# voutcn/megahit

Hardware: NVIDIA H100
Metric: sorted (k+1)-mer edges/sec at k=27 on 150bp reads (higher is better)
Workload: dtype u32

## Files before the change

megahit_b200/csrc/mhb_count.cuh:

```cuda
#pragma once
#include <stdlib.h>
#include <string.h>

#include "mhb.h"
#include "mhb_kernels.cuh"

namespace mhb {

static constexpr int kReadsPerBatch = 64;
static constexpr int kStageWords = 4096;
static constexpr int kExtractThreads = 256;

struct ReadsView {
  const u32 *bin;
  u64 bin_words;
  u64 n_reads;
  u32 fixed_len;
  u32 fixed_stride;
  const u64 *rec_off;
  const u64 *edge_off;
  __device__ __forceinline__ u64 rec_start(u64 r) const { return fixed_len ? r * fixed_stride : rec_off[r]; }
};

template <class F>
__device__ __forceinline__ void for_each_read(const ReadsView &rv, F &&f) {
  __shared__ __align__(16) u32 s_stage[2][kStageWords];
  __shared__ __align__(8) u64 s_bar[2];
  const u32 tid = threadIdx.x, warp = tid >> 5;
  constexpr int NW = kExtractThreads / 32;
  const u64 n_batches = (rv.n_reads + kReadsPerBatch - 1) / kReadsPerBatch;
  if (tid == 0) {
    mbar_init(&s_bar[0], 1);
    mbar_init(&s_bar[1], 1);
    mbar_fence_init();
  }
  __syncthreads();

  auto geom = [&](u64 b, u64 &r0, u64 &r1, u64 &a0, u64 &a1) {
    r0 = b * kReadsPerBatch;
    r1 = r0 + kReadsPerBatch < rv.n_reads ? r0 + kReadsPerBatch : rv.n_reads;
    const u64 w0 = rv.rec_start(r0);
    const u64 w1 = r1 < rv.n_reads ? rv.rec_start(r1) : rv.bin_words;
    a0 = w0 & ~3ull;
    a1 = (w1 + 3) & ~3ull;
  };
  auto issue = [&](u64 b, int st) {
    u64 r0, r1, a0, a1;
    geom(b, r0, r1, a0, a1);
    if (a1 - a0 <= (u64)kStageWords && tid == 0) {
      const u32 bytes = (u32)(a1 - a0) * 4;
      mbar_expect_tx(&s_bar[st], bytes);
      bulk_g2s(&s_stage[st][0], rv.bin + a0, bytes, &s_bar[st]);
    }
  };

  u32 parity[2] = {0, 0};
  u64 b = blockIdx.x;
  int st = 0;
  if (b < n_batches) issue(b, 0);
  for (; b < n_batches; b += gridDim.x, st ^= 1) {
    const u64 nb = b + gridDim.x;
    if (nb < n_batches) issue(nb, st ^ 1);
    u64 r0, r1, a0, a1;
    geom(b, r0, r1, a0, a1);
    const bool staged = (a1 - a0) <= (u64)kStageWords;
    if (staged) {
      mbar_wait(&s_bar[st], parity[st]);
      parity[st] ^= 1;
    }
    for (u64 r = r0 + warp; r < r1; r += NW) {
      const u64 w = rv.rec_start(r);
      const u32 *rec = staged ? &s_stage[st][w - a0] : rv.bin + w;
      const u32 L = rec[0];
      f(r, rec + 1, div_ceil(L, 16), L);
    }
    __syncthreads();
  }
}

template <int W, int WR>
__global__ void __launch_bounds__(kExtractThreads)
    k_count_extract(ReadsView rv, u32 k, u32 *__restrict__ records, u64 *hist, int hist_byte) {
  __shared__ u32 s_hist[256];
  for (int i = threadIdx.x; i < 256; i += kExtractThreads) s_hist[i] = 0;
  const u32 lane = lane_id();
  const u32 K1 = k + 1;
  for_each_read(rv, [&](u64 r, const u32 *s, u32 nwords, u32 L) {
    if (L < K1) return;
    const u32 n_e = L - k;
    const u64 base = rv.fixed_len ? r * (u64)(rv.fixed_len - k) : rv.edge_off[r];
    for (u32 q0 = 0; q0 < n_e; q0 += 32) {
      const u32 q = q0 + lane;
      if (q < n_e) {
        u32 rec[WR], strand;
        make_count_record<W, WR>(s, nwords, L, k, q, rec, strand);
        st_rec<WR>(records, base + q, rec);
        if (hist) atomicAdd(&s_hist[rec_byte<WR>(rec, hist_byte)], 1u);
      }
    }
  });
  __syncthreads();
  if (hist)
    for (int i = threadIdx.x; i < 256; i += kExtractThreads)
      if (s_hist[i]) atomicAdd((unsigned long long *)&hist[i], (unsigned long long)s_hist[i]);
}

static __global__ void __launch_bounds__(kExtractThreads)
    k_count_extract_roll(ReadsView rv, u32 k, u32 *__restrict__ records, u64 *hist, int hist_byte) {
  __shared__ u32 s_hist[256];
  for (int i = threadIdx.x; i < 256; i += kExtractThreads) s_hist[i] = 0;
  const u32 lane = lane_id();
  const u32 K1 = k + 1;
  const u32 hshift = 8u * (u32)hist_byte;
  for_each_read(rv, [&](u64 r, const u32 *s, u32 nwords, u32 L) {
    if (L < K1) return;
    const u32 n_e = L - k;
    const u64 base = rv.fixed_len ? r * (u64)(rv.fixed_len - k) : rv.edge_off[r];
    for (u32 q0 = 0; q0 < n_e; q0 += 128) {
      const u32 q = q0 + 4 * lane;
      if (q < n_e) {
        u64 rec[4];
        u32 strand[4];
        make_count_records_roll<4>(s, nwords, L, k, q, rec, strand);
        const u32 cnt = n_e - q < 4u ? n_e - q : 4u;
#pragma unroll
        for (int j = 0; j < 4; ++j) {
          if ((u32)j < cnt) {
            reinterpret_cast<uint2 *>(records)[base + q + j] = make_uint2((u32)(rec[j] >> 32), (u32)rec[j]);
            if (hist) atomicAdd(&s_hist[(u32)(rec[j] >> hshift) & 255u], 1u);
          }
        }
      }
    }
  });
  __syncthreads();
  if (hist)
    for (int i = threadIdx.x; i < 256; i += kExtractThreads)
      if (s_hist[i]) atomicAdd((unsigned long long *)&hist[i], (unsigned long long)s_hist[i]);
}

template <int W, int WR, bool WRITE>
__global__ void __launch_bounds__(kExtractThreads)
    k_count_extract_range(ReadsView rv, u32 k, u32 lo, u32 hi, u64 *__restrict__ per_read, u32 *__restrict__ records,
                          u64 *hist, int hist_byte) {
  __shared__ u32 s_hist[256];
  for (int i = threadIdx.x; i < 256; i += kExtractThreads) s_hist[i] = 0;
  const u32 lane = lane_id();
  const u32 lt_mask = lanemask_lt();
  const u32 K1 = k + 1;
  for_each_read(rv, [&](u64 r, const u32 *s, u32 nwords, u32 L) {
    if (L < K1) {
      if (!WRITE && lane == 0) per_read[r] = 0;
      return;
    }
    const u32 n_e = L - k;
    u64 run = WRITE ? per_read[r] : 0ull;
    for (u32 q0 = 0; q0 < n_e; q0 += 32) {
      const u32 q = q0 + lane;
      u32 rec[WR], strand;
      bool in = false;
      if (q < n_e) {
        make_count_record<W, WR>(s, nwords, L, k, q, rec, strand);
        const u32 top = rec[0] >> 16;
        in = top >= lo && top <= hi;
      }
      const u32 mask = __ballot_sync(0xffffffffu, in);
      if (in) {
        if constexpr (WRITE) st_rec<WR>(records, run + __popc(mask & lt_mask), rec);
        if (hist) atomicAdd(&s_hist[rec_byte<WR>(rec, hist_byte)], 1u);
      }
      run += __popc(mask);
    }
    if (!WRITE && lane == 0) per_read[r] = run;
  });
  __syncthreads();
  if (hist)
    for (int i = threadIdx.x; i < 256; i += kExtractThreads)
      if (s_hist[i]) atomicAdd((unsigned long long *)&hist[i], (unsigned long long)s_hist[i]);
}

enum { kCountOwnHist = 0, kCountOwnWrite = 1 };
template <int W, int WR, int MODE>
__global__ void __launch_bounds__(kExtractThreads)
    k_count_extract_owners(ReadsView rv, u32 k, unsigned long long *__restrict__ hist16, OwnerSink sink,
                           const u32 *__restrict__ round_lo, const u32 *__restrict__ round_hi) {
  const u32 lane = lane_id(), lt = lanemask_lt();
  const u32 K1 = k + 1;
  for_each_read(rv, [&](u64, const u32 *s, u32 nwords, u32 L) {
    if (L < K1) return;
    const u32 n_e = L - k;
    for (u32 q0 = 0; q0 < n_e; q0 += 32) {
      const u32 q = q0 + lane;
      u32 rec[WR], strand;
      bool in = q < n_e;
      u32 b = 0xFFFFFFFFu;
      if (in) {
        make_count_record<W, WR>(s, nwords, L, k, q, rec, strand);
        b = rec[0] >> 16;
      }
      if constexpr (MODE == kCountOwnHist) {
        const u32 peers = __match_any_sync(0xffffffffu, b);
        if (in && lane == (u32)__ffs(peers) - 1) atomicAdd(hist16 + b, (unsigned long long)__popc(peers));
      } else {
        if (in) {
          const u32 o = __ldg(sink.owner + (b >> 8));
          in = b >= __ldg(round_lo + o) && b <= __ldg(round_hi + o);
        }
        const u32 mask = __ballot_sync(0xffffffffu, in);
        if (mask) sink.template put<WR>(in, rec, mask, lane, lt);
      }
    }
  });
}

template <int WR>
__device__ __forceinline__ bool same_edge(const u32 (&a)[WR], const u32 (&b)[WR]) {
  bool eq = true;
#pragma unroll
  for (int j = 0; j < WR; ++j) {
    const u32 m = (j == WR - 1) ? ~63u : ~0u;
    eq = eq && ((a[j] & m) == (b[j] & m));
  }
  return eq;
}

static constexpr int kMulHistSmem = 1024;

static __global__ void __launch_bounds__(1024) k_scan_u64(u64 *v, u64 nb, u64 *total_out) {
  __shared__ u64 s_w[33];
  __shared__ u64 s_carry;
  if (threadIdx.x == 0) s_carry = 0;
  __syncthreads();
  const u32 lane = lane_id(), warp = threadIdx.x >> 5;
  for (u64 base = 0; base < nb; base += 1024) {
    const u64 i = base + threadIdx.x;
    const u64 x = i < nb ? v[i] : 0;
    u64 inc = x;
#pragma unroll
    for (int d = 1; d < 32; d <<= 1) {
      u64 t = __shfl_up_sync(0xffffffffu, inc, d);
      if (lane >= (u32)d) inc += t;
    }
    if (lane == 31) s_w[warp] = inc;
    __syncthreads();
    if (warp == 0) {
      u64 w = s_w[lane], winc = w;
#pragma unroll
      for (int d = 1; d < 32; d <<= 1) {
        u64 t = __shfl_up_sync(0xffffffffu, winc, d);
        if (lane >= (u32)d) winc += t;
      }
      s_w[lane] = winc - w;
      if (lane == 31) s_w[32] = winc;
    }
    __syncthreads();
    if (i < nb) v[i] = s_carry + s_w[warp] + inc - x;
    __syncthreads();
    if (threadIdx.x == 0) s_carry += s_w[32];
    __syncthreads();
  }
  if (threadIdx.x == 0 && total_out) *total_out = s_carry;
}

struct TipsetHeader {
  u64 capacity;
  u64 filter_words;
  u32 fold;
  u32 filter_bits;
  u32 resident;
  u32 reserved;
};
static_assert(sizeof(TipsetHeader) == 32, "tip set header");
static constexpr u64 kTipFilterSmemWords = 224 * 1024 / 4;
static constexpr u64 kTipMul = 0x9E3779B97F4A7C15ull;

struct TipsetPlan {
  u64 capacity, filter_words;
  u32 fold, filter_bits, resident;
  __host__ __device__ u64 global_words() const { return fold * filter_words; }
  __host__ __device__ u64 folded_words() const { return fold > 1 ? filter_words : 0; }
};

inline TipsetPlan tipset_plan(u64 n_tip, const char *spec) {
  TipsetPlan p;
  p.capacity = 1024;
  while (p.capacity < 2 * n_tip) p.capacity <<= 1;
  char *end = nullptr;
  const unsigned long long forced = spec && *spec ? strtoull(spec, &end, 10) : 0ull;
  if (forced > 0 && end && *end == '\0') {
    p.filter_words = (forced + 3) & ~3ull;
// ... 688 lines not shown
```

megahit_b200/csrc/mhb_device.cu:

```cuda
#include <cuda_runtime.h>
#include <stdarg.h>
#include <stdio.h>
#include <stdlib.h>
#include <string.h>

#include "mhb.h"
#include "mhb_count.cuh"
#include "mhb_internal.h"
#include "mhb_mercy.cuh"
#include "mhb_s2s.cuh"
#include "mhb_common.cuh"

using namespace mhb;

static thread_local char g_err[1024] = "";
int mhb_set_error(int code, const char *fmt, ...) {
  va_list ap;
  va_start(ap, fmt);
  vsnprintf(g_err, sizeof(g_err), fmt, ap);
  va_end(ap);
  return code;
}
extern "C" const char *mhb_last_error(void) { return g_err; }
extern "C" const char *mhb_version(void) { return "megahit_b200 0.1 (sm_90a; formats of megahit v1.2.9)"; }
extern "C" int mhb_device_count(void) {
  int n = 0;
  if (cudaGetDeviceCount(&n) != cudaSuccess) {
    cudaGetLastError();
    return 0;
  }
  return n;
}
extern "C" void mhb_free(void *p) { free(p); }
unsigned long long g_mhb_launches = 0;
extern "C" uint64_t mhb_launch_count(void) { return g_mhb_launches; }


extern "C" uint32_t mhb_count_record_words(uint32_t k) { return count_record_words(k); }
extern "C" uint32_t mhb_words_per_edge(uint32_t k) { return words_per_edge(k); }
extern "C" uint32_t mhb_s2s_record_words(uint32_t k) { return s2s_record_words(k); }

extern "C" uint32_t mhb_count_sort_bytes(uint32_t k, uint8_t *bytes) {
  const u32 wr = count_record_words(k), total_bits = 32 * wr, key_bits = 2 * (k + 1);
  const u32 lo = (total_bits - key_bits) / 8;
  u32 n = 0;
  for (u32 b = lo; b < 4 * wr; ++b) bytes[n++] = (uint8_t)b;
  return n;
}
extern "C" uint32_t mhb_s2s_sort_bytes(uint32_t k, uint8_t *bytes) {
  const u32 w = s2s_record_words(k), total_bits = 32 * w, key_bits = 2 * k;
  const u32 lo = (total_bits - key_bits) / 8;
  u32 n = 0;
  for (u32 b = 2; b < 4 * w; ++b)
    if (b == 2 || b >= lo) bytes[n++] = (uint8_t)b;
  return n;
}


static int g_sm_count = 0;
static int g_bound_device = -1;
int mhb_sm_count() {
  if (!g_sm_count) {
    int dev = 0;
    cudaGetDevice(&dev);
    cudaDeviceGetAttribute(&g_sm_count, cudaDevAttrMultiProcessorCount, dev);
    if (g_sm_count <= 0) g_sm_count = 132;
    if (g_bound_device < 0) g_bound_device = dev;
  }
  return g_sm_count;
}

ReadsView make_reads_view(const mhb_dev_reads *r) {
  ReadsView v;
  v.bin = r->bin;
  v.bin_words = r->bin_words;
  v.n_reads = r->n_reads;
  v.fixed_len = r->fixed_len;
  v.fixed_stride = r->fixed_len ? 1 + div_ceil(r->fixed_len, 16) : 0;
  v.rec_off = r->rec_off;
  v.edge_off = r->edge_off;
  return v;
}

int check_reads(const mhb_dev_reads *r, uint32_t k) {
  if (!r || k < 1 || k > MHB_MAX_K) return mhb_set_error(MHB_ERR_ARG, "bad reads/k (k=%u)", k);
  if (r->n_reads && !r->bin) return mhb_set_error(MHB_ERR_ARG, "reads->bin is NULL");
  if (((uintptr_t)r->bin & 15) != 0) return mhb_set_error(MHB_ERR_ARG, "reads->bin must be 16-byte aligned");
  if (!r->fixed_len && r->n_reads && (!r->rec_off || !r->edge_off))
    return mhb_set_error(MHB_ERR_ARG, "variable-length reads need rec_off and edge_off");
  return MHB_OK;
}

static int grow_scratch(size_t bytes, void **out) {
  static void *buf[64] = {nullptr};
  static size_t cap[64] = {0};
  int dev = 0;
  CK(cudaGetDevice(&dev));
  if (dev < 0 || dev >= 64) return mhb_set_error(MHB_ERR_CUDA, "device index %d out of range", dev);
  if (cap[dev] < bytes) {
    CK(cudaDeviceSynchronize());
    if (buf[dev]) cudaFree(buf[dev]);
    buf[dev] = nullptr;
    cap[dev] = 0;
    const size_t want = (bytes + 4095) & ~(size_t)4095;
    CK(cudaMalloc(&buf[dev], want));
    cap[dev] = want;
  }
  *out = buf[dev];
  return MHB_OK;
}
static int scan64(cudaStream_t st, u64 *v, u64 n, u64 *total_dev, u64 *bsum);

static __global__ void k_check_fixed_len(const u32 *__restrict__ bin, u64 n_reads, u32 stride, u32 L, unsigned long long *flag) {
  bool bad = false;
  for (u64 r = (u64)blockIdx.x * blockDim.x + threadIdx.x; r < n_reads; r += (u64)gridDim.x * blockDim.x) bad |= bin[r * stride] != L;
  if (__any_sync(0xffffffffu, bad) && (threadIdx.x & 31) == 0) atomicOr(flag, 1ull);
}
extern "C" int mhb_check_fixed_len(void *stream, const uint32_t *bin_dev, uint64_t n_reads, uint32_t fixed_len, uint64_t *flag_dev) {
  if (n_reads == 0) return MHB_OK;
  if (!bin_dev || !flag_dev || !fixed_len) return mhb_set_error(MHB_ERR_ARG, "bad arguments");
  k_check_fixed_len<<<mhb_sm_count() * 8, 256, 0, (cudaStream_t)stream>>>(bin_dev, n_reads, 1 + div_ceil(fixed_len, 16), fixed_len,
                                                                     (unsigned long long *)flag_dev);
  CK_LAUNCH();
  return MHB_OK;
}

extern "C" int mhb_count_extract(void *stream, const mhb_dev_reads *reads, uint32_t k, uint32_t *records,
                                 uint64_t n_edges, uint64_t *hist256, int hist_byte) {
  if (int rc = check_reads(reads, k)) return rc;
  if (reads->n_reads == 0 || n_edges == 0) return MHB_OK;
  cudaStream_t st = (cudaStream_t)stream;
  const ReadsView rv = make_reads_view(reads);
  const u32 W = count_key_words(k), WR = count_record_words(k);
  const int grid = (int)grid_cap(rv.n_reads, kReadsPerBatch, 8);
  static const bool roll = getenv("MHB_EXTRACT_ROLL") && !strcmp(getenv("MHB_EXTRACT_ROLL"), "1");
  if (roll && W == 2 && WR == 2 && k + 1 >= 17) {
    k_count_extract_roll<<<grid, kExtractThreads, 0, st>>>(rv, k, records, hist256, hist_byte);
    CK_LAUNCH();
    return MHB_OK;
  }
#define M(WW)                                                                                              \
  if (W == WW && WR == WW)                                                                                 \
    k_count_extract<WW, WW><<<grid, kExtractThreads, 0, st>>>(rv, k, records, hist256, hist_byte);         \
  else if (W == WW && WR == WW + 1)                                                                        \
    k_count_extract<WW, WW + 1><<<grid, kExtractThreads, 0, st>>>(rv, k, records, hist256, hist_byte);     \
  else
  MHB_FOR_W(M) return mhb_set_error(MHB_ERR_ARG, "unsupported k=%u", k);
#undef M
  CK_LAUNCH();
  return MHB_OK;
}

extern "C" int mhb_count_extract_range(void *stream, const mhb_dev_reads *reads, uint32_t k, uint32_t lo, uint32_t hi,
                                       int write, uint64_t *per_read, uint32_t *records, uint64_t *hist256, int hist_byte,
                                       uint64_t *total_dev) {
  if (int rc = check_reads(reads, k)) return rc;
  if (lo > hi || hi > 65535) return mhb_set_error(MHB_ERR_ARG, "bad bucket range [%u, %u]", lo, hi);
  if (!per_read || (write && !records) || (!write && !total_dev)) return mhb_set_error(MHB_ERR_ARG, "null buffer");
  cudaStream_t st = (cudaStream_t)stream;
  if (reads->n_reads == 0) {
    if (!write) CK(cudaMemsetAsync(total_dev, 0, 8, st));
    return MHB_OK;
  }
  const ReadsView rv = make_reads_view(reads);
  const u32 W = count_key_words(k), WR = count_record_words(k);
  const int grid = (int)grid_cap(rv.n_reads, kReadsPerBatch, 8);
#define M2(WW, WRR)                                                                                                   \
  if (W == WW && WR == WRR) {                                                                                         \
    if (write)                                                                                                        \
      k_count_extract_range<WW, WRR, true><<<grid, kExtractThreads, 0, st>>>(rv, k, lo, hi, per_read, records, hist256, hist_byte); \
    else                                                                                                              \
      k_count_extract_range<WW, WRR, false><<<grid, kExtractThreads, 0, st>>>(rv, k, lo, hi, per_read, records, hist256, hist_byte); \
  } else
#define M(WW) M2(WW, WW) M2(WW, WW + 1)
  MHB_FOR_W(M) return mhb_set_error(MHB_ERR_ARG, "unsupported k=%u", k);
#undef M
#undef M2
  CK_LAUNCH();
  if (!write) {
    u64 *bsum = nullptr;
    if (int rc = grow_scratch(((rv.n_reads / kScanTile) + 2) * 8, (void **)&bsum)) return rc;
    if (int rc = scan64(st, per_read, rv.n_reads, total_dev, bsum)) return rc;
    CK(cudaMemcpyAsync(per_read + rv.n_reads, total_dev, 8, cudaMemcpyDeviceToDevice, st));
  }
  return MHB_OK;
}

extern "C" int mhb_count_extract_owners(void *stream, const mhb_dev_reads *reads, uint32_t k, uint64_t *hist16,
                                        const uint8_t *owner_of_byte, const uint64_t *owner_base, uint64_t *cursor_dev,
                                        const uint64_t *capacity_dev, const uint32_t *round_lo, const uint32_t *round_hi) {
  if (int rc = check_reads(reads, k)) return rc;
  if (!hist16 && (!owner_of_byte || !owner_base || !cursor_dev || !capacity_dev || !round_lo || !round_hi))
    return mhb_set_error(MHB_ERR_ARG, "bad args");
  if (reads->n_reads == 0) return MHB_OK;
  cudaStream_t st = (cudaStream_t)stream;
  const ReadsView rv = make_reads_view(reads);
  const u32 W = count_key_words(k), WR = count_record_words(k);
  const int grid = (int)grid_cap(rv.n_reads, kReadsPerBatch, 8);
  const OwnerSink sink{owner_of_byte, owner_base, (unsigned long long *)cursor_dev, capacity_dev};
  unsigned long long *h = (unsigned long long *)hist16;
#define M2(WW, WRR)                                                                                                         \
  if (W == WW && WR == WRR) {                                                                                               \
    if (hist16)                                                                                                             \
      k_count_extract_owners<WW, WRR, kCountOwnHist><<<grid, kExtractThreads, 0, st>>>(rv, k, h, sink, round_lo, round_hi);  \
    else                                                                                                                    \
      k_count_extract_owners<WW, WRR, kCountOwnWrite><<<grid, kExtractThreads, 0, st>>>(rv, k, h, sink, round_lo, round_hi); \
  } else
#define M(WW) M2(WW, WW) M2(WW, WW + 1)
  MHB_FOR_W(M) return mhb_set_error(MHB_ERR_ARG, "unsupported k=%u", k);
#undef M
#undef M2
  CK_LAUNCH();
  return MHB_OK;
}

extern "C" int mhb_count_solid(void *stream, const uint32_t *sorted_records, uint64_t n, uint32_t k, int32_t m,
                               uint32_t *edges_out, uint8_t *aux_out, uint64_t capacity_edges, uint64_t *mul_hist,
                               uint64_t *n_solid_out, void *scratch, size_t scratch_bytes) {
  if (k < 1 || k > MHB_MAX_K || !mul_hist || !n_solid_out) return mhb_set_error(MHB_ERR_ARG, "bad args");
  if (n == 0) return MHB_OK;
  const size_t need = mhb_count_solid_scratch_bytes(n);
  if (scratch_bytes < need) return mhb_set_error(MHB_ERR_ARG, "count scratch too small (%zu < %zu)", scratch_bytes, need);
  cudaStream_t st = (cudaStream_t)stream;
  const u32 WR = count_record_words(k);
  {
#define M(WW)                                                                                                          \
  if (WR == WW) {                                                                                                      \
    constexpr int CH = 32 * count3_ipl(WW);                                                                            \
    const u64 n_chunks = (n + CH - 1) / CH;                                                                            \
    if (n_chunks >= (1ull << 32)) return mhb_set_error(MHB_ERR_ARG, "too many records for one count launch");          \
    const u64 n_sblk = (n_chunks + kScanTile - 1) / kScanTile;                                                         \
    char *p = (char *)scratch;                                                                                         \
    u32 *ticket = (u32 *)p;                                                                                            \
    p += 256;                                                                                                          \
    uint2 *solid_list = (uint2 *)p;                                                                                    \
    p += pad256((size_t)n_chunks * CH * 8);                                                                            \
    u32 *chunk_count = (u32 *)p;                                                                                       \
    p += pad256((size_t)n_chunks * 4);                                                                                 \
    u64 *chunk_off = (u64 *)p;                                                                                         \
    p += pad256((size_t)n_chunks * 8);                                                                                 \
    u64 *bsum = (u64 *)p;                                                                                              \
    CK(cudaMemsetAsync(ticket, 0, 256, st));                                                                           \
    const size_t smem = (size_t)kCount3Warps * count3_warp_words(WW) * 4;                                              \
    static int bps = 0;                                                                                                \
    if (!bps) {                                                                                                        \
      CK(cudaFuncSetAttribute(k_count_lanes<WW>, cudaFuncAttributeMaxDynamicSharedMemorySize, (int)smem));             \
      CK(cudaOccupancyMaxActiveBlocksPerMultiprocessor(&bps, k_count_lanes<WW>, kCount3Warps * 32, smem));             \
      if (bps < 1) bps = 1;                                                                                            \
    }                                                                                                                  \
    u64 grid = (u64)sm_count() * bps;                                                                                  \
    if (grid > (n_chunks + kCount3Warps - 1) / kCount3Warps) grid = (n_chunks + kCount3Warps - 1) / kCount3Warps;      \
    k_count_lanes<WW><<<(unsigned)grid, kCount3Warps * 32, smem, st>>>(sorted_records, n, k, m, (u32)n_chunks, ticket,  \
                                                                      solid_list, chunk_count, mul_hist);             \
    CK_LAUNCH();                                                                                                       \
    k_scan32_sums<<<(unsigned)n_sblk, kScanThreads, 0, st>>>(chunk_count, n_chunks, bsum);                             \
    CK_LAUNCH();                                                                                                       \
    k_scan_u64<<<1, 1024, 0, st>>>(bsum, n_sblk, n_solid_out);                                                         \
    CK_LAUNCH();                                                                                                       \
    k_scan32_apply<<<(unsigned)n_sblk, kScanThreads, 0, st>>>(chunk_count, n_chunks, bsum, chunk_off);                 \
    CK_LAUNCH();                                                                                                       \
    k_count_write<WW><<<grid_cap(n_chunks, 8, 16), 256, 0, st>>>(sorted_records, k, (u32)n_chunks, solid_list, chunk_count, \
                                                    chunk_off, edges_out, aux_out, capacity_edges);                   \
  }
    MHB_FOR_WR(M)
#undef M
    CK_LAUNCH();
    return MHB_OK;
  }
  return mhb_set_error(MHB_ERR_ARG, "unsupported k=%u", k);
}

extern "C" size_t mhb_count_solid_scratch_bytes(uint64_t n) {
  return (size_t)(n + 1024) * 8 + (size_t)(n / 128 + 2) * 12 + (size_t)(n / 128 / kScanTile + 2) * 8 + 4096;
}

static TipsetPlan tipset_plan_env(uint64_t n_tip) { return tipset_plan(n_tip, getenv("MHB_TIPSET_FILTER")); }

extern "C" size_t mhb_tipset_bytes(uint64_t n_tip_edges, uint32_t k) {
  const TipsetPlan p = tipset_plan_env(n_tip_edges);
  return sizeof(TipsetHeader) + (p.global_words() + p.folded_words()) * 4 +
         p.capacity * (size_t)tipset_slot_words(count_key_words(k)) * 4;
}

static int small_scratch(unsigned long long **out) {
  static unsigned long long *buf[64] = {nullptr};
  int dev = 0;
  CK(cudaGetDevice(&dev));
  if (dev < 0 || dev >= 64) return mhb_set_error(MHB_ERR_CUDA, "device index %d out of range", dev);
  if (!buf[dev]) CK(cudaMalloc((void **)&buf[dev], 256));
  *out = buf[dev];
  return MHB_OK;
}

extern "C" int mhb_count_tip_edges(void *stream, const uint8_t *aux, uint64_t n_solid, uint64_t *n_tip_host) {
  cudaStream_t st = (cudaStream_t)stream;
  unsigned long long *d = nullptr;
  *n_tip_host = 0;
  if (n_solid == 0) return MHB_OK;
  if (int rc = small_scratch(&d)) return rc;
  CK(cudaMemsetAsync(d, 0, 8, st));
  k_count_tips<<<sm_count() * 4, 256, 0, st>>>(aux, n_solid, d);
  CK_LAUNCH();
  CK(cudaMemcpyAsync(n_tip_host, d, 8, cudaMemcpyDeviceToHost, st));
// ... 475 lines not shown
```

megahit_b200/csrc/mhb_kernels.cuh:

```cuda
#pragma once
#include <cuda_runtime.h>
#include <stdint.h>

#include "mhb_bits.cuh"

namespace mhb {

static constexpr u32 kSentinel = 4;


template <int W, int WR>
MHB_HD void make_count_record(const u32 *s, u32 nwords, u32 L, u32 k, u32 q, u32 (&rec)[WR], u32 &strand) {
  const u32 K1 = k + 1;
  u32 prev_pkg, next_pkg;
  bool st;
  if constexpr (W == 2) {
    const u32 w0 = q >> 4, sh = (q & 15) * 2;
    const u32 x0 = s[w0];
    const u32 x1 = (w0 + 1 < nwords) ? s[w0 + 1] : 0u;
    const u32 x2 = (w0 + 2 < nwords) ? s[w0 + 2] : 0u;
    const u32 pi = q + K1;
    const u32 pw = ((pi >> 4) == w0 + 1) ? x1 : x2;
    prev_pkg = (pi < L) ? ((pw >> (30 - 2 * (pi & 15))) & 3u) : kSentinel;
    const u32 nwd = (q & 15) ? x0 : (q ? s[w0 - 1] : 0u);
// ... 67 lines not shown

template <int W>
MHB_HD void make_s2s_record(const u32 *s, u32 nwords, u32 L, u32 k, u32 strand, u32 offset, u32 mult,
                            u32 (&rec)[W]) {
  const u32 nc = k - ((offset + k > L) ? 1u : 0u);
  const u32 counting = (offset > 0 && offset + k <= L) ? mult : 0u;
  u32 prev;
  if (strand == 0) {
    prev = offset == 0 ? kSentinel : base_at(s, offset - 1);
    load_sub<W>(s, nwords, offset, nc, rec);
  } else {
    prev = offset == 0 ? kSentinel : 3u - base_at(s, L - offset);
    int off2 = (int)L - (int)k - (int)offset;
    if (off2 < 0) off2 = 0;
    u32 S[W], T[W];
    load_sub<W>(s, nwords, (u32)off2, nc, S);
    reverse_sub<W>(S, nc, T);
    complement_sub<W>(T, nc, rec);
  }
  rec[W - 1] |= ((nc == k) ? 1u : 0u) << 19;
  rec[W - 1] |= prev << 16;
  rec[W - 1] |= 65535u - counting;
}

template <int W>
MHB_HD u64 s2s_local_key(const u32 (&r)[W], u32 k) {
  u32 w2 = 0;
  if constexpr (W >= 3) w2 = r[2];
  const u64 top = ((u64)r[0] << 48) | ((u64)r[1] << 16) | (w2 >> 16);
  const u32 kb = 2 * k - 16;
  const u64 flags = (r[W - 1] >> 16) & 15u;
  return (top & ~(~0ull >> kb)) | (flags << (60 - kb));
}

#if defined(__CUDACC__)
template <int WR>
__device__ __forceinline__ void ld_rec(const u32 *base, u64 idx, u32 (&r)[WR]) {
  if constexpr (WR % 4 == 0) {
    const uint4 *p = reinterpret_cast<const uint4 *>(base + idx * WR);
#pragma unroll
    for (int j = 0; j < WR / 4; ++j) {
      const uint4 v = p[j];
      r[4 * j] = v.x;
      r[4 * j + 1] = v.y;
      r[4 * j + 2] = v.z;
      r[4 * j + 3] = v.w;
    }
  } else if constexpr (WR % 2 == 0) {
    const uint2 *p = reinterpret_cast<const uint2 *>(base + idx * WR);
#pragma unroll
    for (int j = 0; j < WR / 2; ++j) {
      const uint2 v = p[j];
      r[2 * j] = v.x;
      r[2 * j + 1] = v.y;
    }
  } else {
    const u32 *p = base + idx * WR;
#pragma unroll
    for (int j = 0; j < WR; ++j) r[j] = p[j];
  }
}
template <int WR>
__device__ __forceinline__ void st_rec(u32 *base, u64 idx, const u32 (&r)[WR]) {
  if constexpr (WR % 4 == 0) {
    uint4 *p = reinterpret_cast<uint4 *>(base + idx * WR);
#pragma unroll
    for (int j = 0; j < WR / 4; ++j) p[j] = make_uint4(r[4 * j], r[4 * j + 1], r[4 * j + 2], r[4 * j + 3]);
  } else if constexpr (WR % 2 == 0) {
    uint2 *p = reinterpret_cast<uint2 *>(base + idx * WR);
#pragma unroll
    for (int j = 0; j < WR / 2; ++j) p[j] = make_uint2(r[2 * j], r[2 * j + 1]);
  } else {
    u32 *p = base + idx * WR;
#pragma unroll
    for (int j = 0; j < WR; ++j) p[j] = r[j];
  }
}

template <int WR>
__device__ __forceinline__ u32 rec_byte(const u32 (&r)[WR], int b) {
  return (pick<WR>(r, (u32)(WR - 1 - (b >> 2))) >> (8 * (b & 3))) & 255u;
}

template <int W>
__global__ void k_bucket_bounds(const u32 *__restrict__ recs, u64 n, u64 *__restrict__ bounds) {
  const u32 b = blockIdx.x * blockDim.x + threadIdx.x;
  if (b > 65536u) return;
  u64 lo = 0, hi = n;
  while (lo < hi) {
    const u64 mid = (lo + hi) >> 1;
    if ((recs[mid * W] >> 16) < b) lo = mid + 1;
    else hi = mid;
  }
  bounds[b] = lo;
}

__device__ __forceinline__ u32 lane_id() { return threadIdx.x & 31; }
__device__ __forceinline__ u32 lanemask_lt() {
  u32 m;
  asm("mov.u32 %0, %%lanemask_lt;" : "=r"(m));
  return m;
}

struct OwnerSink {
  const uint8_t *owner;
  const u64 *base;
  unsigned long long *cursor;
  const u64 *capacity;
  template <int W>
  __device__ __forceinline__ void put(bool in, const u32 (&rec)[W], u32, u32 lane, u32 lt) const {
    const u32 o = in ? (u32)__ldg(owner + (rec[0] >> 24)) : 0xFFFFFFFFu;
    const u32 peers = __match_any_sync(0xffffffffu, o);
    if (!in) return;
    const u32 leader = (u32)__ffs(peers) - 1;
    unsigned long long at = 0;
    if (lane == leader) at = atomicAdd(cursor + o, (unsigned long long)__popc(peers));
    at = __shfl_sync(peers, at, leader);
    const u64 pos = at + __popc(peers & lt);
    if (pos < capacity[o]) st_rec<W>(reinterpret_cast<u32 *>(base[o]), pos, rec);
  }
};

__device__ __forceinline__ u32 smem_u32(const void *p) { return (u32)__cvta_generic_to_shared(p); }
__device__ __forceinline__ void mbar_init(u64 *bar, u32 count) {
  asm volatile("mbarrier.init.shared::cta.b64 [%0], %1;" ::"r"(smem_u32(bar)), "r"(count) : "memory");
}
__device__ __forceinline__ void mbar_fence_init() {
  asm volatile("fence.mbarrier_init.release.cluster;" ::: "memory");
  asm volatile("fence.proxy.async.shared::cta;" ::: "memory");
}
__device__ __forceinline__ void mbar_expect_tx(u64 *bar, u32 bytes) {
  asm volatile("mbarrier.arrive.expect_tx.shared::cta.b64 _, [%0], %1;" ::"r"(smem_u32(bar)), "r"(bytes)
               : "memory");
}
__device__ __forceinline__ void bulk_g2s(void *dst, const void *src, u32 bytes, u64 *bar) {
  asm volatile("cp.async.bulk.shared::cluster.global.mbarrier::complete_tx::bytes [%0], [%1], %2, [%3];" ::"r"(
                   smem_u32(dst)),
               "l"(src), "r"(bytes), "r"(smem_u32(bar))
               : "memory");
}
__device__ __forceinline__ bool mbar_try_wait(u64 *bar, u32 parity) {
  u32 ok;
  asm volatile(
      "{\n\t.reg .pred p;\n\tmbarrier.try_wait.parity.shared::cta.b64 p, [%1], %2;\n\tselp.u32 %0, 1, 0, p;\n\t}"
      : "=r"(ok)
      : "r"(smem_u32(bar)), "r"(parity)
      : "memory");
  return ok != 0;
}
__device__ __forceinline__ void mbar_wait(u64 *bar, u32 parity) {
  while (!mbar_try_wait(bar, parity)) {
  }
}

__device__ __forceinline__ u64 ld_relaxed(const u64 *p) {
  u64 v;
  asm volatile("ld.relaxed.gpu.global.u64 %0, [%1];" : "=l"(v) : "l"(p) : "memory");
  return v;
}
__device__ __forceinline__ void st_relaxed(u64 *p, u64 v) {
  asm volatile("st.relaxed.gpu.global.u64 [%0], %1;" ::"l"(p), "l"(v) : "memory");
}

static constexpr u64 kLbPartial = 1ull << 62, kLbInclusive = 2ull << 62, kLbStatusMask = 3ull << 62;
static constexpr u64 kLbValueMask = (1ull << 54) - 1;
__host__ __device__ inline u64 lb_epoch(u32 e) { return (u64)(e & 255u) << 54; }

template <int THREADS>
__device__ __forceinline__ u32 block_excl_scan(u32 v, u32 *s_warp , u32 &total) {
  const u32 lane = lane_id(), warp = threadIdx.x >> 5;
  u32 inc = v;
#pragma unroll
  for (int d = 1; d < 32; d <<= 1) {
    u32 t = __shfl_up_sync(0xffffffffu, inc, d);
    if (lane >= (u32)d) inc += t;
  }
  if (lane == 31) s_warp[warp] = inc;
  __syncthreads();
  if (warp == 0) {
    u32 w = lane < THREADS / 32 ? s_warp[lane] : 0u;
    u32 winc = w;
#pragma unroll
    for (int d = 1; d < 32; d <<= 1) {
      u32 t = __shfl_up_sync(0xffffffffu, winc, d);
      if (lane >= (u32)d) winc += t;
    }
    if (lane < THREADS / 32) s_warp[lane] = winc - w;
    if (lane == 31) s_warp[THREADS / 32] = winc;
  }
  __syncthreads();
  u32 res = s_warp[warp] + inc - v;
  total = s_warp[THREADS / 32];
  __syncthreads();
  return res;
}
#endif

}
```

Measured before the change: 18.75 billion.

## Rewrite count extraction with TMA staging, warp-private output buffers and bulk stores

Replaces the extract kernels with one kernel that keeps a 3-stage ring of input batches, loaded by cp.async.bulk with full/empty mbarriers. Each warp writes its records into a double-buffered shared-memory output area and flushes them to global memory with bulk shared-to-global copies, fixing up the unaligned head and tail. Each warp also takes a contiguous range of reads, and for k=27 the rolling path processes two reads per warp step, one per half-warp. The goal is to turn scattered 8-byte stores into large coalesced bulk writes, overlap input loads with compute, and improve lane utilisation on 150bp reads; the cost is much more shared memory, which can lower occupancy, and more complex synchronisation.

```diff
diff --git a/megahit_b200/csrc/mhb_count.cuh b/megahit_b200/csrc/mhb_count.cuh
--- a/megahit_b200/csrc/mhb_count.cuh
+++ b/megahit_b200/csrc/mhb_count.cuh
@@ -78,64 +78,211 @@
   }
 }
 
+static constexpr int kExtThreads = 256;
+static constexpr int kExtWarps = kExtThreads / 32;
+static constexpr int kExtInStages = 3;
+static constexpr int kExtInWords = 2048;
+static constexpr int kExtOutBytes = 3072;
+static constexpr int kExtOutStride = kExtOutBytes + 16;
+static constexpr int kExtHistBytes = 1024, kExtBarBytes = 64;
+static constexpr int kExtSmemBytes =
+    kExtHistBytes + kExtBarBytes + kExtInStages * kExtInWords * 4 + kExtWarps * 2 * kExtOutStride;
+static_assert(2 * kExtInStages * 8 <= kExtBarBytes && kExtOutStride % 16 == 0, "extract shared-memory layout");
+
+__host__ __device__ inline u32 extract_reads_per_batch(u64 n_reads, u64 bin_words, u32 fixed_stride) {
+  const u64 stride = fixed_stride ? fixed_stride : (n_reads ? (bin_words + n_reads - 1) / n_reads : 1);
+  const u64 room = fixed_stride ? (u64)kExtInWords - 6 : (u64)kExtInWords / 2;
+  const u64 r = stride ? room / stride : room;
+  return r < 1 ? 1u : (u32)r;
+}
+
 template <int W, int WR>
-__global__ void __launch_bounds__(kExtractThreads)
-    k_count_extract(ReadsView rv, u32 k, u32 *__restrict__ records, u64 *hist, int hist_byte) {
-  __shared__ u32 s_hist[256];
-  for (int i = threadIdx.x; i < 256; i += kExtractThreads) s_hist[i] = 0;
-  const u32 lane = lane_id();
+__global__ void __launch_bounds__(kExtThreads)
+    k_count_extract(ReadsView rv, u32 k, u32 rpb, u32 *__restrict__ records, u64 *hist, int hist_byte) {
+  extern __shared__ __align__(16) unsigned char ext_smem[];
+  constexpr bool kRoll = W == 2 && WR == 2;
+  constexpr u32 SR = kRoll ? 128 : 32;
+  constexpr u32 CAP = kExtOutBytes / (4 * WR);
+  constexpr u32 kPairEdges = 128;
+  static_assert(CAP >= SR && (!kRoll || CAP >= 2 * kPairEdges), "an output buffer holds a warp step");
+  u32 *s_hist = reinterpret_cast<u32 *>(ext_smem);
+  u64 *full = reinterpret_cast<u64 *>(ext_smem + kExtHistBytes);
+  u64 *empty = full + kExtInStages;
+  u32 *s_in = reinterpret_cast<u32 *>(ext_smem + kExtHistBytes + kExtBarBytes);
+  const u32 tid = threadIdx.x, lane = lane_id(), warp = tid >> 5;
+  unsigned char *s_out = ext_smem + kExtHistBytes + kExtBarBytes + kExtInStages * kExtInWords * 4 + warp * 2 * kExtOutStride;
+  for (int i = tid; i < 256; i += kExtThreads) s_hist[i] = 0;
+  if (tid == 0) {
+    for (int s = 0; s < kExtInStages; ++s) {
+      mbar_init(&full[s], 1);
+      mbar_init(&empty[s], kExtWarps);
+    }
+    mbar_fence_init();
+  }
+  __syncthreads();
+
   const u32 K1 = k + 1;
-  for_each_read(rv, [&](u64 r, const u32 *s, u32 nwords, u32 L) {
-    if (L < K1) return;
-    const u32 n_e = L - k;
-    const u64 base = rv.fixed_len ? r * (u64)(rv.fixed_len - k) : rv.edge_off[r];
-    for (u32 q0 = 0; q0 < n_e; q0 += 32) {
-      const u32 q = q0 + lane;
-      if (q < n_e) {
-        u32 rec[WR], strand;
-        make_count_record<W, WR>(s, nwords, L, k, q, rec, strand);
-        st_rec<WR>(records, base + q, rec);
-        if (hist) atomicAdd(&s_hist[rec_byte<WR>(rec, hist_byte)], 1u);
-      }
-    }
-  });
+  const u64 n_batches = (rv.n_reads + rpb - 1) / rpb;
+  auto geom = [&](u64 b, u64 &r0, u64 &r1, u64 &a0, u64 &a1) {
+    r0 = b * rpb;
+    r1 = r0 + rpb < rv.n_reads ? r0 + rpb : rv.n_reads;
+    const u64 w0 = rv.rec_start(r0);
+    const u64 w1 = r1 < rv.n_reads ? rv.rec_start(r1) : rv.bin_words;
+    a0 = w0 & ~3ull;
+    a1 = (w1 + 3) & ~3ull;
+  };
+  auto issue = [&](u64 i) {
+    const u64 b = blockIdx.x + i * gridDim.x;
+    if (b >= n_batches) return;
+    const u32 st = (u32)(i % kExtInStages);
+    if (i >= (u64)kExtInStages) mbar_wait(&empty[st], (u32)((i / kExtInStages - 1) & 1));
+    u64 r0, r1, a0, a1;
+    geom(b, r0, r1, a0, a1);
+    if (a1 - a0 <= (u64)kExtInWords) {
+      const u32 bytes = (u32)(a1 - a0) * 4;
+      mbar_expect_tx(&full[st], bytes);
+      bulk_g2s(s_in + st * kExtInWords, rv.bin + a0, bytes, &full[st]);
+    } else {
+      mbar_expect_tx(&full[st], 0);
+    }
+  };
+
+  u32 cur = 0, n = 0, o = 0;
+  u64 d0 = 0;
+  auto flush = [&]() {
+    const u32 *sw = reinterpret_cast<const u32 *>(s_out + cur * kExtOutStride + o);
+    u32 *g = records + d0 * WR;
+    const u32 nw = n * WR;
+    const u32 h = min(((16u - o) & 15u) >> 2, nw);
+    const u32 body = (nw - h) & ~3u;
+    const u32 tail = nw - h - body;
+    fence_proxy_async_smem();
+    __syncwarp();
+    if (lane == 0) {
+      if (body) {
+        bulk_s2g(g + h, sw + h, body * 4);
+        bulk_commit();
+        bulk_wait_read<1>();
+      } else {
+        bulk_wait_read<0>();
+      }
+    }
+    if (lane < h) g[lane] = sw[lane];
+    else if (lane >= 4 && lane - 4 < tail) g[h + body + lane - 4] = sw[h + body + lane - 4];
+    __syncwarp();
+    cur ^= 1;
+    n = 0;
+  };
+  auto reserve = [&](u64 dst, u32 cnt) -> u32 * {
+    if (n && (dst != d0 + n || n + cnt > CAP)) flush();
+    if (n == 0) {
+      d0 = dst;
+      o = (u32)(reinterpret_cast<uintptr_t>(records + dst * WR) & 15u);
+    }
+    return reinterpret_cast<u32 *>(s_out + cur * kExtOutStride + o);
+  };
+
+  if (tid == 0)
+    for (int i = 0; i < kExtInStages - 1; ++i) issue(i);
+  for (u64 i = 0;; ++i) {
+    const u64 b = blockIdx.x + i * gridDim.x;
+    if (b >= n_batches) break;
+    if (tid == 0) issue(i + kExtInStages - 1);
+    const u32 st = (u32)(i % kExtInStages);
+    mbar_wait(&full[st], (u32)((i / kExtInStages) & 1));
+    u64 r0, r1, a0, a1;
+    geom(b, r0, r1, a0, a1);
+    const bool staged = a1 - a0 <= (u64)kExtInWords;
+    const u64 nr = r1 - r0;
+    const u64 my0 = r0 + nr * warp / kExtWarps, my1 = r0 + nr * (warp + 1) / kExtWarps;
+    auto read_words = [&](u64 r) -> const u32 * {
+      const u64 w = rv.rec_start(r);
+      return staged ? s_in + st * kExtInWords + (w - a0) : rv.bin + w;
+    };
+    for (u64 r = my0; r < my1; ++r) {
+      const u32 *rec0 = read_words(r);
+      const u32 L = rec0[0];
+      if constexpr (kRoll) {
+        if (r + 1 < my1) {
+          const u32 *rec1 = read_words(r + 1);
+          const u32 L1 = rec1[0];
+          const u32 ne0 = L >= K1 ? L - k : 0u, ne1 = L1 >= K1 ? L1 - k : 0u;
+          if (ne0 <= kPairEdges && ne1 <= kPairEdges) {
+            const u32 cnt = ne0 + ne1;
+            if (cnt) {
+              const u64 dst = rv.fixed_len ? r * (u64)(rv.fixed_len - k) : rv.edge_off[r];
+              u32 *buf = reserve(dst, cnt);
+              const u32 half = lane >> 4;
+              const u32 Lh = half ? L1 : L, ne = half ? ne1 : ne0;
+              const u32 q = 8 * (lane & 15);
+              if (q < ne) {
+                u64 rec[8];
+                u32 strand[8];
+                make_count_records_roll<8>((half ? rec1 : rec0) + 1, div_ceil(Lh, 16), Lh, k, q, rec, strand);
+                const u32 c = ne - q < 8u ? ne - q : 8u;
+                const u32 at = (u32)(dst - d0) + (half ? ne0 : 0u) + q;
+                const u32 hshift = 8u * (u32)hist_byte;
+#pragma unroll
+                for (int j = 0; j < 8; ++j) {
+                  if ((u32)j < c) {
+                    reinterpret_cast<uint2 *>(buf)[at + j] = make_uint2((u32)(rec[j] >> 32), (u32)rec[j]);
+                    if (hist) red_shared_add(&s_hist[(u32)(rec[j] >> hshift) & 255u], 1u);
+                  }
+                }
+              }
+              n += cnt;
+            }
+            ++r;
+            continue;
+          }
+        }
+      }
+      if (L < K1) continue;
+      const u32 *s = rec0 + 1;
+      const u32 nwords = div_ceil(L, 16);
+      const u32 n_e = L - k;
+      const u64 base = rv.fixed_len ? r * (u64)(rv.fixed_len - k) : rv.edge_off[r];
+      for (u32 q0 = 0; q0 < n_e; q0 += SR) {
+        const u32 cnt = n_e - q0 < SR ? n_e - q0 : SR;
+        const u64 dst = base + q0;
+        u32 *buf = reserve(dst, cnt);
+        const u32 at = (u32)(dst - d0);
+        if constexpr (kRoll) {
+          const u32 q = q0 + 4 * lane;
+          if (q < n_e) {
+            u64 rec[4];
+            u32 strand[4];
+            make_count_records_roll<4>(s, nwords, L, k, q, rec, strand);
+            const u32 c = n_e - q < 4u ? n_e - q : 4u;
+            const u32 hshift = 8u * (u32)hist_byte;
+#pragma unroll
+            for (int j = 0; j < 4; ++j) {
+              if ((u32)j < c) {
+                reinterpret_cast<uint2 *>(buf)[at + 4 * lane + j] = make_uint2((u32)(rec[j] >> 32), (u32)rec[j]);
+                if (hist) red_shared_add(&s_hist[(u32)(rec[j] >> hshift) & 255u], 1u);
+              }
+            }
+          }
+        } else {
+          const u32 q = q0 + lane;
+          if (q < n_e) {
+            u32 rec[WR], strand;
+            make_count_record<W, WR>(s, nwords, L, k, q, rec, strand);
+            st_rec<WR>(buf, at + lane, rec);
+            if (hist) red_shared_add(&s_hist[rec_byte<WR>(rec, hist_byte)], 1u);
+          }
+        }
+        n += cnt;
+      }
+    }
+    __syncwarp();
+    if (lane == 0) mbar_arrive(&empty[st]);
+  }
+  if (n) flush();
+  if (lane == 0) bulk_wait_all();
   __syncthreads();
   if (hist)
-    for (int i = threadIdx.x; i < 256; i += kExtractThreads)
-      if (s_hist[i]) atomicAdd((unsigned long long *)&hist[i], (unsigned long long)s_hist[i]);
-}
-
-static __global__ void __launch_bounds__(kExtractThreads)
-    k_count_extract_roll(ReadsView rv, u32 k, u32 *__restrict__ records, u64 *hist, int hist_byte) {
-  __shared__ u32 s_hist[256];
-  for (int i = threadIdx.x; i < 256; i += kExtractThreads) s_hist[i] = 0;
-  const u32 lane = lane_id();
-  const u32 K1 = k + 1;
-  const u32 hshift = 8u * (u32)hist_byte;
-  for_each_read(rv, [&](u64 r, const u32 *s, u32 nwords, u32 L) {
-    if (L < K1) return;
-    const u32 n_e = L - k;
-    const u64 base = rv.fixed_len ? r * (u64)(rv.fixed_len - k) : rv.edge_off[r];
-    for (u32 q0 = 0; q0 < n_e; q0 += 128) {
-      const u32 q = q0 + 4 * lane;
-      if (q < n_e) {
-        u64 rec[4];
-        u32 strand[4];
-        make_count_records_roll<4>(s, nwords, L, k, q, rec, strand);
-        const u32 cnt = n_e - q < 4u ? n_e - q : 4u;
-#pragma unroll
-        for (int j = 0; j < 4; ++j) {
-          if ((u32)j < cnt) {
-            reinterpret_cast<uint2 *>(records)[base + q + j] = make_uint2((u32)(rec[j] >> 32), (u32)rec[j]);
-            if (hist) atomicAdd(&s_hist[(u32)(rec[j] >> hshift) & 255u], 1u);
-          }
-        }
-      }
-    }
-  });
-  __syncthreads();
-  if (hist)
-    for (int i = threadIdx.x; i < 256; i += kExtractThreads)
+    for (int i = tid; i < 256; i += kExtThreads)
       if (s_hist[i]) atomicAdd((unsigned long long *)&hist[i], (unsigned long long)s_hist[i]);
 }
 
diff --git a/megahit_b200/csrc/mhb_device.cu b/megahit_b200/csrc/mhb_device.cu
--- a/megahit_b200/csrc/mhb_device.cu
+++ b/megahit_b200/csrc/mhb_device.cu
@@ -125,6 +125,20 @@
   return MHB_OK;
 }
 
+template <int W, int WR>
+static int launch_extract(cudaStream_t st, const ReadsView &rv, u32 k, u32 *records, u64 *hist256, int hist_byte) {
+  CK(cudaFuncSetAttribute(k_count_extract<W, WR>, cudaFuncAttributeMaxDynamicSharedMemorySize, kExtSmemBytes));
+  int per_sm = 0;
+  CK(cudaOccupancyMaxActiveBlocksPerMultiprocessor(&per_sm, k_count_extract<W, WR>, kExtThreads, kExtSmemBytes));
+  const u32 rpb = extract_reads_per_batch(rv.n_reads, rv.bin_words, rv.fixed_stride);
+  const u64 n_batches = (rv.n_reads + rpb - 1) / rpb;
+  const u64 cap = (u64)mhb_sm_count() * (u64)(per_sm > 0 ? per_sm : 1);
+  const int grid = (int)(n_batches < cap ? n_batches : cap);
+  k_count_extract<W, WR><<<grid, kExtThreads, kExtSmemBytes, st>>>(rv, k, rpb, records, hist256, hist_byte);
+  CK_LAUNCH();
+  return MHB_OK;
+}
+
 extern "C" int mhb_count_extract(void *stream, const mhb_dev_reads *reads, uint32_t k, uint32_t *records,
                                  uint64_t n_edges, uint64_t *hist256, int hist_byte) {
   if (int rc = check_reads(reads, k)) return rc;
@@ -132,23 +146,14 @@
   cudaStream_t st = (cudaStream_t)stream;
   const ReadsView rv = make_reads_view(reads);
   const u32 W = count_key_words(k), WR = count_record_words(k);
-  const int grid = (int)grid_cap(rv.n_reads, kReadsPerBatch, 8);
-  static const bool roll = getenv("MHB_EXTRACT_ROLL") && !strcmp(getenv("MHB_EXTRACT_ROLL"), "1");
-  if (roll && W == 2 && WR == 2 && k + 1 >= 17) {
-    k_count_extract_roll<<<grid, kExtractThreads, 0, st>>>(rv, k, records, hist256, hist_byte);
-    CK_LAUNCH();
-    return MHB_OK;
-  }
-#define M(WW)                                                                                              \
-  if (W == WW && WR == WW)                                                                                 \
-    k_count_extract<WW, WW><<<grid, kExtractThreads, 0, st>>>(rv, k, records, hist256, hist_byte);         \
-  else if (W == WW && WR == WW + 1)                                                                        \
-    k_count_extract<WW, WW + 1><<<grid, kExtractThreads, 0, st>>>(rv, k, records, hist256, hist_byte);     \
+#define M(WW)                                                                                \
+  if (W == WW && WR == WW)                                                                   \
+    return launch_extract<WW, WW>(st, rv, k, records, hist256, hist_byte);                   \
+  else if (W == WW && WR == WW + 1)                                                          \
+    return launch_extract<WW, WW + 1>(st, rv, k, records, hist256, hist_byte);               \
   else
   MHB_FOR_W(M) return mhb_set_error(MHB_ERR_ARG, "unsupported k=%u", k);
 #undef M
-  CK_LAUNCH();
-  return MHB_OK;
 }
 
 extern "C" int mhb_count_extract_range(void *stream, const mhb_dev_reads *reads, uint32_t k, uint32_t lo, uint32_t hi,
diff --git a/megahit_b200/csrc/mhb_kernels.cuh b/megahit_b200/csrc/mhb_kernels.cuh
--- a/megahit_b200/csrc/mhb_kernels.cuh
+++ b/megahit_b200/csrc/mhb_kernels.cuh
@@ -243,6 +243,23 @@
   while (!mbar_try_wait(bar, parity)) {
   }
 }
+__device__ __forceinline__ void mbar_arrive(u64 *bar) {
+  asm volatile("mbarrier.arrive.shared::cta.b64 _, [%0];" ::"r"(smem_u32(bar)) : "memory");
+}
+__device__ __forceinline__ void fence_proxy_async_smem() { asm volatile("fence.proxy.async.shared::cta;" ::: "memory"); }
+__device__ __forceinline__ void bulk_s2g(void *dst, const void *src, u32 bytes) {
+  asm volatile("cp.async.bulk.global.shared::cta.bulk_group [%0], [%1], %2;" ::"l"(dst), "r"(smem_u32(src)), "r"(bytes)
+               : "memory");
+}
+__device__ __forceinline__ void bulk_commit() { asm volatile("cp.async.bulk.commit_group;" ::: "memory"); }
+template <int N>
+__device__ __forceinline__ void bulk_wait_read() {
+  asm volatile("cp.async.bulk.wait_group.read %0;" ::"n"(N) : "memory");
+}
+__device__ __forceinline__ void bulk_wait_all() { asm volatile("cp.async.bulk.wait_group 0;" ::: "memory"); }
+__device__ __forceinline__ void red_shared_add(u32 *p, u32 v) {
+  asm volatile("red.shared.add.u32 [%0], %1;" ::"r"(smem_u32(p)), "r"(v) : "memory");
+}
 
 __device__ __forceinline__ u64 ld_relaxed(const u64 *p) {
   u64 v;
```

Result: faster. 19.20 billion, median of 6 (+2.4%).
